# snakers4/silero-vad

Hardware: AMD Instinct MI355X
Metric: audio-chunks/sec (32 ms @ 16 kHz) (higher is better)
Workload: dtype f32; 1 GPU; configs[1]: synthetic 16 kHz PCM resident in HBM, 512-sample chunks, 4096 streams/GPU x 256 chunks/stream per step, zero initial state; streams_per_gpu=4096

## Files before the change

### silero_vad_amd/csrc/fft_wave.hpp

```cpp
#pragma once
#include <hip/hip_runtime.h>

#include "device_api.hpp"
#include "layout.hpp"

#ifndef VAD_NT_PCM
#define VAD_NT_PCM 0
#endif

namespace vad {
namespace {

using f32x4 = float __attribute__((ext_vector_type(4)));
using u32x4 = unsigned __attribute__((ext_vector_type(4)));

#ifndef VAD_TRACE
#define VAD_TRACE 0
#endif
#ifndef VAD_ABLATE
#define VAD_ABLATE 0
#endif

__device__ constexpr float kCos32[16] = {1.0f, 0.98078525f, 0.9238795f, 0.8314696f, 0.70710677f,
    0.55557024f, 0.38268343f, 0.19509032f, 0.0f, -0.19509032f, -0.38268343f, -0.55557024f,
    -0.70710677f, -0.8314696f, -0.9238795f, -0.98078525f};
__device__ constexpr float kSin32[16] = {0.0f, 0.19509032f, 0.38268343f, 0.55557024f, 0.70710677f,
    0.8314696f, 0.9238795f, 0.98078525f, 1.0f, 0.98078525f, 0.9238795f, 0.8314696f, 0.70710677f,
    0.55557024f, 0.38268343f, 0.19509032f};

constexpr int bitrev(int x, int bits) {
    int r = 0;
    for (int i = 0; i < bits; ++i) r |= ((x >> i) & 1) << (bits - 1 - i);
    return r;
}
constexpr int ilog2(int x) { return x <= 1 ? 0 : 1 + ilog2(x / 2); }

struct Lane {
    int lane, g, j, wave;
    long t;
    long tl;
    long st;
    int b;
    bool tile_valid;
    bool from_tail;
    float sgnA, sgnB;
#if VAD_TRACE
    mutable unsigned long long ts[20] = {};
#endif
};
#if VAD_TRACE
#define VAD_WAVE_STAMP(ln, slot) do { (ln).ts[(slot)] = __builtin_readcyclecounter(); } while (0)
#else
#define VAD_WAVE_STAMP(ln, slot) do { } while (0)
#endif

__device__ __forceinline__ void cvt8(const u32x4 v, float *o) {
#pragma unroll
    for (int k = 0; k < 4; ++k) {
        const int lo = (int)(v[k] << 16) >> 16, hi = (int)v[k] >> 16;
        o[2 * k] = (float)lo * (1.0f / 32768.0f);
        o[2 * k + 1] = (float)hi * (1.0f / 32768.0f);
    }
}
template <int SL, int DEC>
__device__ __forceinline__ void load_vec(const float *p, float (&s)[SL]) {
    if (DEC == 1) {
#pragma unroll
        for (int k = 0; k < SL / 4; ++k) {
            const f32x4 v = VAD_NT_PCM ? __builtin_nontemporal_load(reinterpret_cast<const f32x4 *>(p) + k)
                                       : reinterpret_cast<const f32x4 *>(p)[k];
#pragma unroll
            for (int e = 0; e < 4; ++e) s[4 * k + e] = v[e];
        }
    } else {
#pragma unroll
        for (int i = 0; i < SL; ++i) s[i] = p[i * DEC];
        __builtin_amdgcn_sched_barrier(0);
    }
}
template <int SL, int DEC>
__device__ __forceinline__ void load_vec(const int16_t *p, float (&s)[SL]) {
    if (DEC == 1) {
#pragma unroll
        for (int k = 0; k < SL / 8; ++k)
            cvt8(VAD_NT_PCM ? __builtin_nontemporal_load(reinterpret_cast<const u32x4 *>(p) + k)
                            : reinterpret_cast<const u32x4 *>(p)[k], &s[8 * k]);
    } else {
#pragma unroll
        for (int h = 0; h < 2; ++h) {
#pragma unroll
            for (int i = h * SL / 2; i < (h + 1) * SL / 2; ++i) s[i] = (float)p[i * DEC] * (1.0f / 32768.0f);
            __builtin_amdgcn_sched_barrier(0);
        }
    }
}

template <int Q, typename PcmT, int DEC>
__device__ __forceinline__ void load_slice(float (&s)[2 * Q], const FrontArgs &a, const Lane &ln, const int V) {
    constexpr int SL = 2 * Q, N = 16 * Q;
    const PcmT *row = reinterpret_cast<const PcmT *>(a.pcm) + (size_t)ln.b * a.ld;
    const int sigma = 2 * V + ln.g;
    const int sg = (V == 3 && sigma > 8) ? 8 : sigma;
    const long p0 = (long)SL * (8 * ln.t - 1 + sg);
    const PcmT *src = row + p0 * DEC;
    const PcmT *esrc = row + ((long)N * ln.t + N - SL - 1) * DEC;
    if (ln.from_tail) {
        const PcmT *trow = reinterpret_cast<const PcmT *>(a.tail) + (size_t)ln.b * N * DEC;
        if (sg > 0) src = trow + SL * (sg - 1) * DEC;
        esrc = trow + (N - SL - 1) * DEC;
    }
    if (VAD_ABLATE & 16) {
        const PcmT *r0 = reinterpret_cast<const PcmT *>(a.pcm) + (size_t)(ln.st * 16) * a.ld + (long)SL * 8 * ln.t;
#pragma unroll
        for (int k = 0; k < SL / 4; ++k) {
            const f32x4 v = *reinterpret_cast<const f32x4 *>(reinterpret_cast<const float *>(r0) + (size_t)(k & 15) * a.ld + ln.lane * 4);
#pragma unroll
            for (int e = 0; e < 4; ++e) s[4 * k + e] = v[e];
        }
    } else if (VAD_ABLATE & 32) {
        const float *rr = reinterpret_cast<const float *>(row) + (long)SL * 8 * ln.t;
#pragma unroll
        for (int k = 0; k < SL / 4; ++k) {
            const f32x4 v = *reinterpret_cast<const f32x4 *>(rr + 16 * k + 4 * ln.g + 128 * V);
#pragma unroll
            for (int e = 0; e < 4; ++e) s[4 * k + e] = v[e];
        }
    } else if (DEC == 1) {
        if (V == 0 && ln.t == 0 && ln.g == 0) load_vec<SL, 1>(a.ctx_in + (size_t)ln.b * SL, s);
        else load_vec<SL, 1>(src, s);
    } else if (V == 0) {
        const bool from_ctx = ln.t == 0 && ln.g == 0;
        const PcmT *safe = ln.from_tail ? reinterpret_cast<const PcmT *>(a.tail) + (size_t)ln.b * N * DEC : row;
        load_vec<SL, DEC>(from_ctx ? safe : src, s);
        const f32x4 *c4 = reinterpret_cast<const f32x4 *>(a.ctx_in + (size_t)ln.b * SL);
#pragma unroll
        for (int k = 0; k < SL / 4; ++k) {
            const f32x4 v = c4[k];
#pragma unroll
            for (int e = 0; e < 4; ++e) s[4 * k + e] = from_ctx ? v[e] : s[4 * k + e];
        }
    } else {
        load_vec<SL, DEC>(src, s);
    }
    if (V == 3) {
        if (a.ctx_out && ln.t == a.T - 1 && ln.g == 2 && ln.tile_valid &&
            (ln.st * 16 + ln.j) < a.B) {
            float *o = a.ctx_out + (size_t)ln.b * SL;
#pragma unroll
            for (int k = 0; k < SL / 4; ++k)
                reinterpret_cast<f32x4 *>(o)[k] = f32x4{s[4 * k], s[4 * k + 1], s[4 * k + 2], s[4 * k + 3]};
        }
        const bool rev = ln.g == 3;
        float extra = 0.f;
        if (rev) extra = load_pcm(esrc);
#pragma unroll
        for (int i = 0; i < SL / 2 - 1; ++i) {
            const int k = SL - 2 - i;
            const float lo = s[i], hi = s[k];
            s[i] = rev ? hi : lo;
            s[k] = rev ? lo : hi;
        }
        s[SL - 1] = rev ? extra : s[SL - 1];
    }
}

using f32x2 = float __attribute__((ext_vector_type(2)));

__device__ __forceinline__ f32x2 swap2(f32x2 v) { return f32x2{v.y, v.x}; }
__device__ __forceinline__ f32x2 cmul(f32x2 v, float c, float sn) {
    return __builtin_elementwise_fma(swap2(v), f32x2{-sn, sn}, v * f32x2{c, c});
}

#ifndef VAD_XLANE_SWAP
#define VAD_XLANE_SWAP 1
#endif
__device__ __forceinline__ void trade32(f32x2 &a, f32x2 &b) {
#pragma unroll
    for (int e = 0; e < 2; ++e) {
        const auto r = __builtin_amdgcn_permlane32_swap(__float_as_uint(a[e]), __float_as_uint(b[e]), false, false);
        a[e] = __uint_as_float(r[0]);
        b[e] = __uint_as_float(r[1]);
    }
}
__device__ __forceinline__ void trade16(f32x2 &a, f32x2 &b) {
#pragma unroll
    for (int e = 0; e < 2; ++e) {
        const auto r = __builtin_amdgcn_permlane16_swap(__float_as_uint(a[e]), __float_as_uint(b[e]), false, false);
        a[e] = __uint_as_float(r[0]);
        b[e] = __uint_as_float(r[1]);
    }
}

template <int Q>
__device__ __forceinline__ void fft_inlane(f32x2 (&z)[Q]) {
#pragma unroll
    for (int n = Q; n >= 2; n >>= 1) {
        const int half = n >> 1;
#pragma unroll
        for (int b0 = 0; b0 < Q; b0 += n) {
#pragma unroll
            for (int jx = 0; jx < half; ++jx) {
                const int i0 = b0 + jx, i1 = i0 + half;
                const f32x2 u = z[i0], v = z[i1];
                z[i0] = u + v;
                const f32x2 d = u - v;
                const int tw = jx * (32 / n);
                if (tw == 0) z[i1] = d;
                else if (tw == 8) z[i1] = swap2(d) * f32x2{1.0f, -1.0f};
                else z[i1] = cmul(d, kCos32[tw], -kSin32[tw]);
            }
        }
    }
}

template <int Q>
__device__ __forceinline__ void fft_math(float (&X)[Q + 1], const float (&s)[2 * Q], const float *tab_lds, const Lane &ln);

template <int Q, typename PcmT, int DEC = 1>
__device__ __forceinline__ void fft_frame(float (&X)[Q + 1], const int V, const FrontArgs &a, const float *tab_lds,
                                          const Lane &ln) {
    constexpr int SL = 2 * Q;
    __builtin_amdgcn_sched_barrier(0);
    VAD_WAVE_STAMP(ln, 16 + V);
    float s[SL];
    if (VAD_ABLATE & 4) {
#pragma unroll
        for (int i = 0; i < SL; ++i) s[i] = (float)(ln.lane + i) * 1e-3f;
    } else {
        load_slice<Q, PcmT, DEC>(s, a, ln, V);
    }
#if VAD_TRACE
    asm volatile("s_waitcnt vmcnt(0)" ::: "memory");
    VAD_WAVE_STAMP(ln, 2 + 2 * V);
#endif
    if (VAD_ABLATE & 2) {
#pragma unroll
        for (int k = 0; k < Q; ++k) X[k] = s[k] + s[k + Q];
        X[Q] = s[0];
        return;
    }
    fft_math<Q>(X, s, tab_lds, ln);
    VAD_WAVE_STAMP(ln, 3 + 2 * V);
}

template <int Q>
__device__ __forceinline__ void fft_math(float (&X)[Q + 1], const float (&s)[2 * Q], const float *tab_lds, const Lane &ln) {
    constexpr int SL = 2 * Q;
    constexpr vadl::Tab tb = vadl::make_tab(8 * Q, Q);

    f32x2 z[Q];
    {
        const f32x4 *w = reinterpret_cast<const f32x4 *>(tab_lds + tb.window + SL * ln.g);
#pragma unroll
        for (int k = 0; k < SL / 4; ++k) {
            const f32x4 wv = w[k];
            z[2 * k] = f32x2{s[4 * k], s[4 * k + 1]} * f32x2{wv[0], wv[1]};
            z[2 * k + 1] = f32x2{s[4 * k + 2], s[4 * k + 3]} * f32x2{wv[2], wv[3]};
        }
    }
    const f32x4 *tw1 = reinterpret_cast<const f32x4 *>(tab_lds + tb.tw1 + ln.g * Q * 4);
#if VAD_XLANE_SWAP
    constexpr int H = Q / 2;
    const f32x2 rotA = (ln.g & 1) ? f32x2{0.f, 0.f} : f32x2{1.f, 1.f};
    const f32x2 rotB = (ln.g & 1) ? f32x2{1.f, -1.f} : f32x2{0.f, 0.f};
#pragma unroll
    for (int q = 0; q < H; ++q) trade32(z[q], z[q + H]);
#pragma unroll
    for (int q = 0; q < H; ++q) {
        const f32x2 u = z[q], v = z[q + H], d = u - v;
        z[q] = u + v;
        z[q + H] = __builtin_elementwise_fma(swap2(d), rotB, d * rotA);
    }
#pragma unroll
    for (int q = 0; q < H; ++q) trade32(z[q], z[q + H]);
#pragma unroll
    for (int q = 0; q < H; ++q) trade16(z[q], z[q + H]);
#pragma unroll
    for (int q = 0; q < H; ++q) {
        const f32x2 u = z[q], v = z[q + H];
        z[q] = u + v;
        z[q + H] = u - v;
    }
#pragma unroll
    for (int q = 0; q < H; ++q) trade16(z[q], z[q + H]);
#pragma unroll
    for (int q = 0; q < Q; ++q) {
        const f32x2 x = z[q];
        const f32x4 t = tw1[q];
        z[q] = __builtin_elementwise_fma(swap2(x), f32x2{t[0], t[1]}, x * f32x2{t[2], t[2]});
    }
#else
    const f32x2 sA{ln.sgnA, ln.sgnA}, sB{ln.sgnB, ln.sgnB};
    const f32x2 rotA = ln.g == 3 ? f32x2{0.f, 0.f} : f32x2{1.f, 1.f};
    const f32x2 rotB = ln.g == 3 ? f32x2{1.f, -1.f} : f32x2{0.f, 0.f};
#pragma unroll
    for (int q = 0; q < Q; ++q) {
        f32x2 x = z[q];
        const f32x2 p{__shfl_xor(x.x, 32), __shfl_xor(x.y, 32)};
        x = __builtin_elementwise_fma(sA, x, p);
        x = __builtin_elementwise_fma(swap2(x), rotB, x * rotA);
        const f32x2 r{__shfl_xor(x.x, 16), __shfl_xor(x.y, 16)};
        x = __builtin_elementwise_fma(sB, x, r);
        const f32x4 t = tw1[q];
        z[q] = __builtin_elementwise_fma(swap2(x), f32x2{t[0], t[1]}, x * f32x2{t[2], t[2]});
    }
#endif
    fft_inlane<Q>(z);
    constexpr int LG = ilog2(Q);
    const f32x4 *tw2 = reinterpret_cast<const f32x4 *>(tab_lds + tb.tw2 + ln.g * Q * 4);
    const int src_lane4 = (ln.g >= 2 ? (ln.lane ^ 16) : ln.lane) * 4;
#pragma unroll
    for (int k = 0; k < Q; ++k) {
        const f32x2 u = z[bitrev(k, LG)];
        const int ks = bitrev((Q - k) % Q, LG), kr = bitrev(Q - 1 - k, LG);
        const f32x2 own = z[kr], alt = z[ks];
        const float xr = __int_as_float(__builtin_amdgcn_ds_bpermute(src_lane4, __float_as_int(own.x)));
        const float xi = __int_as_float(__builtin_amdgcn_ds_bpermute(src_lane4, __float_as_int(own.y)));
        const f32x2 p{ln.g == 0 ? alt.x : xr, ln.g == 0 ? alt.y : xi};
        const f32x2 av = __builtin_elementwise_fma(p, f32x2{1.0f, -1.0f}, u);
        const f32x2 ev = __builtin_elementwise_fma(p, f32x2{-1.0f, 1.0f}, u);
        const f32x4 t = tw2[k];
        const f32x2 y = __builtin_elementwise_fma(swap2(ev), f32x2{t[0], t[1]},
                                                  __builtin_elementwise_fma(ev, f32x2{t[2], t[2]}, av));
        const f32x2 yy = y * y;
        X[k] = 0.5f * __builtin_amdgcn_sqrtf(yy.x + yy.y);
    }
    X[Q] = ln.g == 0 ? fabsf(z[0].x - z[0].y) : 0.f;
}

template <int Q>
__device__ __forceinline__ void poison_acc(float &p0, float &p1, const float (&X)[Q + 1]) {
#pragma unroll
    for (int k = 0; k < Q; k += 2) {
        p0 = fmaf(X[k], 0.f, p0);
        p1 = fmaf(X[k + 1], 0.f, p1);
    }
}
__device__ __forceinline__ float poison_nyq(float p0, float p1, float xn0, float xn1, float xn2, float xn3) {
    p0 = fmaf(xn0, 0.f, p0);
    p1 = fmaf(xn1, 0.f, p1);
    p0 = fmaf(xn2, 0.f, p0);
    p1 = fmaf(xn3, 0.f, p1);
    return p0 + p1;
}
__device__ __forceinline__ void poison_into(f32x4 &v, float p) {
    v[0] = __uint_as_float(__float_as_uint(v[0]) | __float_as_uint(p));
}

template <int Q, int V, typename PcmT, int DEC = 1>
__device__ __forceinline__ void fft_pass(float (&X)[Q + 1], const FrontArgs &a, const float *tab_lds, const Lane &ln) {
    fft_frame<Q, PcmT, DEC>(X, V, a, tab_lds, ln);
}

}
}
```

### silero_vad_amd/csrc/kernel_front_f43.hip

```cpp
#include <hip/hip_runtime.h>

#include <type_traits>

#include "fft_wave.hpp"
#include "exact_front.hpp"
#include "front_common.hpp"

namespace vad {
namespace {

#ifndef VAD_BV_BATCH
#define VAD_BV_BATCH 1
#endif
constexpr int kUnitBytes = (int)vadl::kWUnitFloats * 4;
struct Ring {
    unsigned a_cur, a_nxt, a_far;
    unsigned d_cur, d_nxt, d_far;
    const float *src;
    unsigned voff;
    f32x4 c0, c1;
};

__device__ __forceinline__ void ring_request(Ring &r) {
    if (VAD_ABLATE & 8) return;
    unsigned keep_m0;
    asm volatile("s_mov_b32 %0, m0\n\ts_mov_b32 m0, %3\n\ts_nop 0\n\t"
                 "global_load_lds_dwordx4 %1, %2\n\tglobal_load_lds_dwordx4 %1, %2 offset:1024\n\t"
                 "global_load_lds_dwordx4 %1, %2 offset:2048\n\tglobal_load_lds_dwordx4 %1, %2 offset:3072\n\t"
                 "s_mov_b32 m0, %0"
                 : "=&s"(keep_m0) : "v"(r.voff), "s"(r.src), "s"(r.d_far) : "memory");
    r.src += vadl::kWUnitFloats;
}
__device__ __forceinline__ void ring_rotate(Ring &r) {
    const unsigned a = r.a_cur, d = r.d_cur;
    r.a_cur = r.a_nxt; r.a_nxt = r.a_far; r.a_far = a;
    r.d_cur = r.d_nxt; r.d_nxt = r.d_far; r.d_far = d;
}

template <int M, int KG, int AFTER, class BF>
__device__ __forceinline__ void gemm_r(f32x4 (&acc)[M], BF bfun, Ring &r) {
    constexpr int NSTEPS = KG * (M / 2), NU = NSTEPS / 8;
    static_assert(NSTEPS % 8 == 0 && M % 2 == 0, "segments are whole units");
    static_for<0, NU>([&](auto uc) VAD_INLINE {
        constexpr int u = decltype(uc)::value, after = (NU - 1 - u) + AFTER;
        static_for<0, 8>([&](auto sc_) VAD_INLINE {
            constexpr int st = decltype(sc_)::value;
            if constexpr (st == 4 && after >= 1) {
                asm volatile("s_waitcnt vmcnt(0)" ::: "memory");
                if (!(VAD_ABLATE & 1)) __builtin_amdgcn_s_barrier();
                asm volatile("" ::: "memory");
                if constexpr (after >= 2) ring_request(r);
            }
            f32x4 n0 = r.c0, n1 = r.c1;
            if constexpr (st + 1 < 8) {
                n0 = lds4(r.a_cur + (2 * (st + 1)) * 1024);
                n1 = lds4(r.a_cur + (2 * (st + 1) + 1) * 1024);
            } else if constexpr (after >= 1) {
                n0 = lds4(r.a_nxt);
                n1 = lds4(r.a_nxt + 1024);
            }
            __builtin_amdgcn_sched_barrier(0);
            constexpr int i = u * 8 + st, kg = i / (M / 2), mp = 2 * (i % (M / 2));
#if VAD_BV_BATCH
            float bv[4];
#pragma unroll
            for (int ks = 0; ks < 4; ++ks) bv[ks] = bfun(kg * 4 + ks);
            __builtin_amdgcn_sched_barrier(0);
#pragma unroll
            for (int ks = 0; ks < 4; ++ks) {
                acc[mp + 0] = __builtin_amdgcn_mfma_f32_16x16x4f32(r.c0[ks], bv[ks], acc[mp + 0], 0, 0, 0);
                acc[mp + 1] = __builtin_amdgcn_mfma_f32_16x16x4f32(r.c1[ks], bv[ks], acc[mp + 1], 0, 0, 0);
            }
#else
#pragma unroll
            for (int ks = 0; ks < 4; ++ks) {
                const float bv = bfun(kg * 4 + ks);
                acc[mp + 0] = __builtin_amdgcn_mfma_f32_16x16x4f32(r.c0[ks], bv, acc[mp + 0], 0, 0, 0);
                acc[mp + 1] = __builtin_amdgcn_mfma_f32_16x16x4f32(r.c1[ks], bv, acc[mp + 1], 0, 0, 0);
            }
#endif
            __builtin_amdgcn_sched_barrier(0);
            r.c0 = n0;
            r.c1 = n1;
        });
        ring_rotate(r);
    });
}

#ifndef VAD_F43_GEMM_PRIO
#define VAD_F43_GEMM_PRIO 0
#endif
#ifndef VAD_F43_FFT_PRIO
#define VAD_F43_FFT_PRIO 0
#endif
template <int Q, typename PcmT, int DEC>
__global__ void __launch_bounds__(256, 2) front_f43_kernel(const FrontArgs a) {
    using namespace vadl;
    constexpr Tab tb = make_tab(8 * Q, Q);
    constexpr int TABF = (tb.total + 3) / 4 * 4;
    constexpr int RB = w_rb(Q), P = w_parts(Q), KG0 = Q / 4;
    constexpr int PB = Q == 32 ? 2 : 1;
    static_assert(w4_tail0(Q) + 20 == w4_units(Q) && P % PB == 0, "program mismatch");
    __shared__ __attribute__((aligned(16))) float lds[TABF + 3 * (kUnitBytes / 4)];
    float *tab = lds;

    Lane ln;
    ln.lane = threadIdx.x & 63;
    ln.wave = __builtin_amdgcn_readfirstlane(threadIdx.x >> 6);
    ln.g = ln.lane >> 4;
    ln.j = ln.lane & 15;
    const long nst = (a.B + 15) / 16, total = nst * a.nt;
    long wt = (long)blockIdx.x * 4 + ln.wave;
    ln.tile_valid = wt < total;
    if (!ln.tile_valid) wt = total - 1;
    ln.tl = wt % a.nt;
    ln.st = wt / a.nt;
    ln.t = a.t0 + ln.tl;
    const long bb = ln.st * 16 + ln.j;
    ln.b = (int)(bb < a.B ? bb : a.B - 1);
    ln.from_tail = a.tail != nullptr && ln.t == a.T - 1;
    ln.sgnA = ln.g < 2 ? 1.f : -1.f;
    ln.sgnB = (ln.g & 1) ? -1.f : 1.f;
#if VAD_TRACE
    VAD_WAVE_STAMP(ln, 0);
#endif

    Ring ring;
    {
        const unsigned slot0 = (unsigned)(size_t)((__attribute__((address_space(3))) float *)(lds + TABF));
        ring.voff = ln.lane * 16;
        ring.a_cur = slot0 + ring.voff;
        ring.a_nxt = ring.a_cur + kUnitBytes;
        ring.a_far = ring.a_cur + 2 * kUnitBytes;
        ring.d_far = slot0 + (unsigned)ln.wave * 4096u;
        ring.d_cur = ring.d_far + kUnitBytes;
        ring.d_nxt = ring.d_far + 2 * kUnitBytes;
        ring.src = a.wfront + ln.wave * 1024;
        ring_request(ring);
        {   const unsigned d = ring.d_far; ring.d_far = ring.d_cur; ring.d_cur = ring.d_nxt; ring.d_nxt = d; }
        ring_request(ring);
        {   const unsigned d = ring.d_far; ring.d_far = ring.d_cur; ring.d_cur = ring.d_nxt; ring.d_nxt = d; }
    }
    {
        static_assert(tb.total % 4 == 0, "tables are copied as 16-byte vectors");
        constexpr int NV = tb.total / 4, PER = (NV + 255) / 256;
        const f32x4 *src = reinterpret_cast<const f32x4 *>(a.tables);
        f32x4 v[PER];
#pragma unroll
        for (int k = 0; k < PER; ++k) {
            const int i = threadIdx.x + k * 256;
            v[k] = src[i < NV ? i : NV - 1];
        }
#pragma unroll
        for (int k = 0; k < PER; ++k) {
            const int i = threadIdx.x + k * 256;
            if (i < NV) reinterpret_cast<f32x4 *>(tab)[i] = v[k];
        }
    }
    asm volatile("s_waitcnt vmcnt(0)" ::: "memory");
    __syncthreads();
    VAD_WAVE_STAMP(ln, 1);

    float X0[Q + 1], X1[Q + 1], X2[Q + 1], X3[Q + 1];
#pragma unroll
    for (int k = 0; k <= Q; ++k) X1[k] = X2[k] = X3[k] = 0.f;
#pragma clang loop unroll(disable)
    for (int v = 0; v < 4; ++v) {
        if (v >= 3) {
#pragma unroll
            for (int k = 0; k <= Q; ++k) X0[k] = X1[k];
        }
        if (v >= 2) {
#pragma unroll
            for (int k = 0; k <= Q; ++k) X1[k] = X2[k];
        }
        if (v >= 1) {
#pragma unroll
            for (int k = 0; k <= Q; ++k) X2[k] = X3[k];
        }
        if (VAD_F43_FFT_PRIO) __builtin_amdgcn_s_setprio(VAD_F43_FFT_PRIO);
        fft_frame<Q, PcmT, DEC>(X3, v, a, tab, ln);
        if (VAD_F43_FFT_PRIO) __builtin_amdgcn_s_setprio(0);
    }
    if (VAD_F43_GEMM_PRIO) __builtin_amdgcn_s_setprio(VAD_F43_GEMM_PRIO);
    const float xn0 = __shfl(X0[Q], ln.j), xn1 = __shfl(X1[Q], ln.j), xn2 = __shfl(X2[Q], ln.j), xn3 = __shfl(X3[Q], ln.j);
    if (!VAD_NO_EXACT && a.exact_list != nullptr) {
        const SilentMasks sm = silent_chunks(X0[0], X1[0], X2[0], X3[0]);
        const long left = (long)a.B - ln.st * 16;
        const unsigned take = (sm.edge | (a.gx_silent != nullptr ? sm.silent : 0u)) & (left >= 16 ? 0xffffu : ((1u << left) - 1u));
        if (take != 0 && ln.tile_valid) {
            int base = 0;
            if (ln.lane == 0) base = atomicAdd(a.exact_list, __builtin_popcount(take));
            base = __shfl(base, 0);
            if (ln.g == 0 && ((take >> ln.j) & 1))
                a.exact_list[2 + base + __builtin_popcount(take & ((1u << ln.j) - 1u))] =
                    (int)(wt * 16 + ln.j) | (((sm.silent >> ln.j) & 1) ? kExactSilentBit : 0);
        }
    }

#if VAD_F43_EF
#pragma unroll
    for (int k = 0; k < Q; ++k) {
        X3[k] = X3[k] - X1[k];
        X0[k] = X2[k] - X0[k];
    }
    float poison;
    {   float p0 = 0.f, p1 = 0.f;
        poison_acc<Q>(p0, p1, X3);
        poison_acc<Q>(p0, p1, X0);
        poison = poison_nyq(p0, p1, xn0, xn1, xn2, xn3);
    }
#else
    float poison;
    {   float p0 = 0.f, p1 = 0.f;
        poison_acc<Q>(p0, p1, X0);
        poison_acc<Q>(p0, p1, X1);
        poison_acc<Q>(p0, p1, X2);
        poison_acc<Q>(p0, p1, X3);
        poison = poison_nyq(p0, p1, xn0, xn1, xn2, xn3);
    }
#endif
    ring.c0 = lds4(ring.a_cur);
    ring.c1 = lds4(ring.a_cur + 1024);

    f32x4 Z0[4], Z1[4];
    zero<4>(Z0);
    zero<4>(Z1);
#pragma clang loop unroll(disable)
    for (int it = 0; it < P / PB; ++it) {
        f32x4 Ykeep[RB];
        static_for<0, PB>([&](auto pc) VAD_INLINE {
            constexpr int pb = decltype(pc)::value;
            const int row0 = 16 * RB * (it * PB + pb);
            const float *wn = tab + tb.w_nyq + row0;
            f32x4 Y0[RB], Y1[RB], Y2[RB], Y3[RB];
            zero<RB>(Y0);
            zero<RB>(Y1);
            zero<RB>(Y2);
            zero<RB>(Y3);
#if VAD_F43_EF
            {   const Coef k = opaque_coef<kF4, kFm3>();
                gemm_r<RB, KG0, 2>(Y0, [&](int s) VAD_INLINE {
                    return fmaf(fmaf(X2[s], k.p1, X1[s]), k.b, fmaf(X0[s], k.a, X3[s])); }, ring);
                const Coef k2 = opaque_coef<kFm4, kF3>();
                gemm_r<RB, KG0, 2>(Y1, [&](int s) VAD_INLINE {
                    return fmaf(fmaf(X1[s], k2.m1, X2[s]), k2.b, fmaf(X0[s], k2.a, X3[s])); }, ring);
            }
            {   const Coef k = opaque_coef<kF2, kFm2>();
                gemm_r<RB, KG0, 2>(Y2, [&](int s) VAD_INLINE { return fmaf(X0[s], k.a, X3[s]); }, ring);
                gemm_r<RB, KG0, 2>(Y3, [&](int s) VAD_INLINE { return fmaf(X0[s], k.b, X3[s]); }, ring);
            }
#else
            {   const Coef k = opaque_coef<kFm4, kF4>();
                gemm_r<RB, KG0, 2>(Y0, [&](int s) VAD_INLINE {
                    return fmaf(fmaf(X1[s], k.p1, X0[s]), k.a, fmaf(X3[s], k.p1, X2[s])); }, ring);
                gemm_r<RB, KG0, 2>(Y1, [&](int s) VAD_INLINE {
                    return fmaf(fmaf(X1[s], k.m1, X0[s]), k.b, fmaf(X2[s], k.m1, X3[s])); }, ring);
            }
            {   const Coef k = opaque_coef<kF2, kFm2>();
                gemm_r<RB, KG0, 2>(Y2, [&](int s) VAD_INLINE {
                    return fmaf(fmaf(X0[s], k.m1, X2[s]), k.a, fmaf(X1[s], k.m1, X3[s])); }, ring);
                const Coef k2 = opaque_coef<kF2, kFm2>();
                gemm_r<RB, KG0, 2>(Y3, [&](int s) VAD_INLINE {
                    return fmaf(fmaf(X0[s], k2.m1, X2[s]), k2.b, fmaf(X1[s], k2.m1, X3[s])); }, ring);
            }
#endif
#pragma unroll
            for (int m = 0; m < RB; ++m)
#pragma unroll
                for (int r = 0; r < 4; ++r) {
                    const float sm = Y0[m][r] + Y1[m][r], df = Y0[m][r] - Y1[m][r];
                    const float s2 = Y2[m][r] + Y3[m][r], d2 = Y2[m][r] - Y3[m][r];
                    Y0[m][r] = sm + s2;
                    Y1[m][r] = fmaf(2.f, d2, df);
                    Y2[m][r] = fmaf(4.f, s2, sm);
                    Y3[m][r] = fmaf(8.f, d2, df);
                }
#if VAD_F43_EF
            {   const Coef k = opaque_coef<kFm4, kFm025>();
                gemm_r<RB, KG0, 2>(Y0, [&](int s) VAD_INLINE { return fmaf(X1[s], k.a, X3[s]); }, ring);
                gemm_r<RB, KG0, 2>(Y3, [&](int s) VAD_INLINE { return fmaf(X2[s], k.b, -X0[s]); }, ring);
            }
#else
            {   const Coef k = opaque_coef<kFm5, kFm125>();
                gemm_r<RB, KG0, 2>(Y0, [&](int s) VAD_INLINE { return fmaf(X1[s], k.a, X3[s]); }, ring);
                gemm_r<RB, KG0, 2>(Y3, [&](int s) VAD_INLINE { return fmaf(X2[s], k.b, X0[s]); }, ring);
            }
#endif
            nyq_update<RB>(Y0, xn0, wn + 128, ln);
            nyq_update<RB>(Y0, xn1, wn + 256, ln);
            nyq_update<RB>(Y1, xn0, wn, ln);
            nyq_update<RB>(Y1, xn1, wn + 128, ln);
            nyq_update<RB>(Y1, xn2, wn + 256, ln);
            nyq_update<RB>(Y2, xn1, wn, ln);
            nyq_update<RB>(Y2, xn2, wn + 128, ln);
            nyq_update<RB>(Y2, xn3, wn + 256, ln);
            nyq_update<RB>(Y3, xn2, wn, ln);
            nyq_update<RB>(Y3, xn3, wn + 128, ln);
            add_bias<RB>(Y0, tab + tb.b_e0 + row0, ln);
            add_bias<RB>(Y1, tab + tb.b_e0 + row0, ln);
            add_bias<RB>(Y2, tab + tb.b_e0 + row0, ln);
            add_bias<RB>(Y3, tab + tb.b_e0 + row0, ln);
            relu<RB>(Y0);
            relu<RB>(Y1);
            relu<RB>(Y2);
            relu<RB>(Y3);
            if constexpr (Q == 32) {
                auto two = [](const f32x4 (&A)[RB], const f32x4 (&B)[RB], int s) VAD_INLINE {
                    return s < 8 ? A[s >> 2][s & 3] : B[(s - 8) >> 2][s & 3];
                };
                gemm_r<4, 4, 2>(Z0, [&](int s) VAD_INLINE { return two(Y0, Y1, s); }, ring);
                gemm_r<4, 4, 2>(Z1, [&](int s) VAD_INLINE { return two(Y1, Y2, s); }, ring);
                if constexpr (pb == 0) {
#pragma unroll
                    for (int m = 0; m < RB; ++m) Ykeep[m] = Y3[m];
                } else {
                    gemm_r<4, 4, 2>(Z1, [&](int s) VAD_INLINE { return two(Ykeep, Y3, s); }, ring);
                }
            } else {
                auto one = [](const f32x4 (&A)[RB], int s) VAD_INLINE { return A[s >> 2][s & 3]; };
                gemm_r<4, 4, 2>(Z0, [&](int s) VAD_INLINE { return one(Y0, s); }, ring);
                gemm_r<4, 4, 2>(Z0, [&](int s) VAD_INLINE { return one(Y1, s); }, ring);
                gemm_r<4, 4, 2>(Z1, [&](int s) VAD_INLINE { return one(Y1, s); }, ring);
                gemm_r<4, 4, 2>(Z1, [&](int s) VAD_INLINE { return one(Y2, s); }, ring);
                gemm_r<4, 4, 2>(Z1, [&](int s) VAD_INLINE { return one(Y3, s); }, ring);
            }
        });
    }
    add_bias<4>(Z0, tab + tb.b_e1, ln);
    add_bias<4>(Z1, tab + tb.b_e1, ln);
    relu<4>(Z0);
    relu<4>(Z1);
    VAD_WAVE_STAMP(ln, 10);

    f32x4 Vv[4];
    auto bZ0 = [&](int s) VAD_INLINE { return Z0[s >> 2][s & 3]; };
    auto bZ1 = [&](int s) VAD_INLINE { return Z1[s >> 2][s & 3]; };
    auto bV = [&](int s) VAD_INLINE { return Vv[s >> 2][s & 3]; };
    init_bias<4>(Vv, tab + tb.b_e2, ln);
    gemm_r<4, 4, 2>(Vv, bZ0, ring);
    gemm_r<4, 4, 2>(Vv, bZ1, ring);
    relu<4>(Vv);
    f32x4 Fe[8];
    auto bF = [&](int s) VAD_INLINE { return Fe[s >> 2][s & 3]; };
    init_bias<8>(Fe, tab + tb.b_e3, ln);
    gemm_r<8, 4, 2>(Fe, bV, ring);
    relu<8>(Fe);
    poison_into(Fe[0], poison);
    VAD_WAVE_STAMP(ln, 11);

    float *gxt = a.gx + ((size_t)(ln.st * a.nt + ln.tl) * 32) * 256 + ln.lane * 4;
    const float *bg = tab + tb.b_g;
#pragma clang loop unroll(disable)
    for (int q = 0; q < 3; ++q) {
        f32x4 G[8];
        init_bias<8>(G, bg, ln);
        gemm_r<8, 8, 2>(G, bF, ring);
        if (ln.tile_valid) {
#pragma unroll
            for (int m = 0; m < 8; ++m) *reinterpret_cast<f32x4 *>(gxt + (size_t)m * 256) = G[m];
        }
        gxt += 8 * 256;
        bg += 128;
    }
    {
        f32x4 G[8];
        init_bias<8>(G, bg, ln);
        gemm_r<8, 8, 0>(G, bF, ring);
        if (ln.tile_valid) {
#pragma unroll
            for (int m = 0; m < 8; ++m) *reinterpret_cast<f32x4 *>(gxt + (size_t)m * 256) = G[m];
        }
    }
#if VAD_TRACE
    VAD_WAVE_STAMP(ln, 12);
    if (a.trace && ln.lane == 0) {
        long long *tr = a.trace + ((size_t)blockIdx.x * 4 + ln.wave) * 32;
#pragma unroll
        for (int k = 0; k < 20; ++k) tr[k] = (long long)ln.ts[k];
        tr[13] = __builtin_amdgcn_s_getreg((31 << 11) | 4);
        tr[14] = __builtin_amdgcn_s_getreg((31 << 11) | 20);
        tr[15] = (long long)wall_clock64();
    }
#endif
}

}

template <typename PcmT>
hipError_t launch_front_f43(int sr, const FrontArgs &a, hipStream_t s) {
    if (a.B <= 0 || a.nt <= 0) return hipSuccess;
    const long nst = (a.B + 15) / 16, total = nst * a.nt;
    const unsigned grid = (unsigned)((total + 3) / 4);
    if (a.dec > 1 && (sr != 16000 || a.dec > 3)) return hipErrorInvalidValue;
    if (a.dec == 3) hipLaunchKernelGGL((front_f43_kernel<32, PcmT, 3>), dim3(grid), dim3(256), 0, s, a);
    else if (a.dec == 2) hipLaunchKernelGGL((front_f43_kernel<32, PcmT, 2>), dim3(grid), dim3(256), 0, s, a);
    else if (sr == 16000) hipLaunchKernelGGL((front_f43_kernel<32, PcmT, 1>), dim3(grid), dim3(256), 0, s, a);
    else hipLaunchKernelGGL((front_f43_kernel<16, PcmT, 1>), dim3(grid), dim3(256), 0, s, a);
    return hipGetLastError();
}
template hipError_t launch_front_f43<float>(int, const FrontArgs &, hipStream_t);
template hipError_t launch_front_f43<int16_t>(int, const FrontArgs &, hipStream_t);

}
```

Before: 189.4 million chunks/s.

## Software-pipeline LDS twiddle/window loads and bpermutes in the FFT front, raise FFT priority

The window, tw1 and tw2 LDS reads and the ds_bpermute exchanges in the per-frame FFT are restructured into batched prefetches with explicit partial lgkmcnt waits, so later batches' LDS traffic overlaps arithmetic on earlier batches. Twiddle rows are loaded as 3-float vectors instead of 4. The FFT wave's priority is now raised only once its PCM global loads have arrived (vmcnt wait inside fft_math), and the default FFT priority becomes 1. This adds register pressure from the staged buffers and depends on hand-coded waitcnt encodings being correct.

```diff
diff --git a/silero_vad_amd/csrc/fft_wave.hpp b/silero_vad_amd/csrc/fft_wave.hpp
--- a/silero_vad_amd/csrc/fft_wave.hpp
+++ b/silero_vad_amd/csrc/fft_wave.hpp
@@ -213,10 +213,10 @@
     }
 }
 
-template <int Q>
+template <int Q, int ARRIVE = -1>
 __device__ __forceinline__ void fft_math(float (&X)[Q + 1], const float (&s)[2 * Q], const float *tab_lds, const Lane &ln);
 
-template <int Q, typename PcmT, int DEC = 1>
+template <int Q, typename PcmT, int DEC = 1, int PRIO = 0>
 __device__ __forceinline__ void fft_frame(float (&X)[Q + 1], const int V, const FrontArgs &a, const float *tab_lds,
                                           const Lane &ln) {
     constexpr int SL = 2 * Q;
@@ -239,26 +239,77 @@
         X[Q] = s[0];
         return;
     }
-    fft_math<Q>(X, s, tab_lds, ln);
+    fft_math<Q, PRIO>(X, s, tab_lds, ln);
+    if (PRIO > 0) __builtin_amdgcn_s_setprio(0);
     VAD_WAVE_STAMP(ln, 3 + 2 * V);
 }
 
-template <int Q>
+__device__ __forceinline__ void lds_fence() { __builtin_amdgcn_sched_barrier(0); }
+template <int N>
+__device__ __forceinline__ void lds_wait() {
+    static_assert(N >= 0 && N <= 15, "lgkmcnt is a 4-bit field");
+    lds_fence();
+    __builtin_amdgcn_s_waitcnt(0xc07f | (N << 8));
+    lds_fence();
+}
+__device__ __forceinline__ void lds_wait_n(int n) {
+    if (n >= 15) lds_wait<15>();
+    else if (n >= 12) lds_wait<12>();
+    else if (n >= 8) lds_wait<8>();
+    else if (n >= 4) lds_wait<4>();
+    else if (n >= 2) lds_wait<2>();
+    else lds_wait<0>();
+}
+template <int N>
+__device__ __forceinline__ void lds_rows(f32x4 (&o)[N], const f32x4 *p) {
+#pragma unroll
+    for (int i = 0; i < N; ++i) o[i] = p[i];
+}
+using f32x3 = float __attribute__((ext_vector_type(3)));
+__device__ __forceinline__ f32x3 tw_row(const f32x4 *p) { return *reinterpret_cast<const f32x3 *>(p); }
+
+template <int Q, int ARRIVE>
 __device__ __forceinline__ void fft_math(float (&X)[Q + 1], const float (&s)[2 * Q], const float *tab_lds, const Lane &ln) {
     constexpr int SL = 2 * Q;
     constexpr vadl::Tab tb = vadl::make_tab(8 * Q, Q);
+    constexpr int TB = 4, NTB = Q / TB, T1B = 4, NT1 = Q / T1B, T1D = 3;
+    static_assert(Q % TB == 0 && SL % 16 == 0, "batches are whole");
+    const f32x4 *tw1 = reinterpret_cast<const f32x4 *>(tab_lds + tb.tw1 + ln.g * Q * 4);
+    const f32x4 *tw2 = reinterpret_cast<const f32x4 *>(tab_lds + tb.tw2 + ln.g * Q * 4);
 
     f32x2 z[Q];
     {
+        constexpr int NWB = 4, WQ = SL / 4 / NWB;
         const f32x4 *w = reinterpret_cast<const f32x4 *>(tab_lds + tb.window + SL * ln.g);
-#pragma unroll
-        for (int k = 0; k < SL / 4; ++k) {
-            const f32x4 wv = w[k];
-            z[2 * k] = f32x2{s[4 * k], s[4 * k + 1]} * f32x2{wv[0], wv[1]};
-            z[2 * k + 1] = f32x2{s[4 * k + 2], s[4 * k + 3]} * f32x2{wv[2], wv[3]};
-        }
-    }
-    const f32x4 *tw1 = reinterpret_cast<const f32x4 *>(tab_lds + tb.tw1 + ln.g * Q * 4);
+        f32x4 wv[NWB][WQ];
+        lds_fence();
+        lds_rows<WQ>(wv[0], w);
+        lds_rows<WQ>(wv[1], w + WQ);
+        if (ARRIVE >= 0) {
+            lds_fence();
+            __builtin_amdgcn_s_waitcnt(0x0f70);
+            if (ARRIVE > 0) __builtin_amdgcn_s_setprio(ARRIVE);
+        }
+#pragma unroll
+        for (int b = 0; b < NWB; ++b) {
+            if (b < NWB - 1) lds_wait<WQ>();
+            else lds_wait<0>();
+#pragma unroll
+            for (int i = 0; i < WQ; ++i) {
+                const int k = b * WQ + i;
+                z[2 * k] = f32x2{s[4 * k], s[4 * k + 1]} * f32x2{wv[b][i][0], wv[b][i][1]};
+                z[2 * k + 1] = f32x2{s[4 * k + 2], s[4 * k + 3]} * f32x2{wv[b][i][2], wv[b][i][3]};
+            }
+            lds_fence();
+            if (b + 2 < NWB) lds_rows<WQ>(wv[b + 2], w + (b + 2) * WQ);
+        }
+    }
+    f32x3 t1[NT1][T1B];
+#pragma unroll
+    for (int b = 0; b < T1D - 1; ++b)
+#pragma unroll
+        for (int i = 0; i < T1B; ++i) t1[b][i] = tw_row(tw1 + b * T1B + i);
+    lds_fence();
 #if VAD_XLANE_SWAP
     constexpr int H = Q / 2;
     const f32x2 rotA = (ln.g & 1) ? f32x2{0.f, 0.f} : f32x2{1.f, 1.f};
@@ -283,12 +334,6 @@
     }
 #pragma unroll
     for (int q = 0; q < H; ++q) trade16(z[q], z[q + H]);
-#pragma unroll
-    for (int q = 0; q < Q; ++q) {
-        const f32x2 x = z[q];
-        const f32x4 t = tw1[q];
-        z[q] = __builtin_elementwise_fma(swap2(x), f32x2{t[0], t[1]}, x * f32x2{t[2], t[2]});
-    }
 #else
     const f32x2 sA{ln.sgnA, ln.sgnA}, sB{ln.sgnB, ln.sgnB};
     const f32x2 rotA = ln.g == 3 ? f32x2{0.f, 0.f} : f32x2{1.f, 1.f};
@@ -300,32 +345,76 @@
         x = __builtin_elementwise_fma(sA, x, p);
         x = __builtin_elementwise_fma(swap2(x), rotB, x * rotA);
         const f32x2 r{__shfl_xor(x.x, 16), __shfl_xor(x.y, 16)};
-        x = __builtin_elementwise_fma(sB, x, r);
-        const f32x4 t = tw1[q];
-        z[q] = __builtin_elementwise_fma(swap2(x), f32x2{t[0], t[1]}, x * f32x2{t[2], t[2]});
-    }
-#endif
+        z[q] = __builtin_elementwise_fma(sB, x, r);
+    }
+#endif
+    lds_fence();
+#pragma unroll
+    for (int b = 0; b < NT1; ++b) {
+        if (b + T1D - 1 < NT1) {
+#pragma unroll
+            for (int i = 0; i < T1B; ++i) t1[b + T1D - 1][i] = tw_row(tw1 + (b + T1D - 1) * T1B + i);
+        }
+        lds_wait_n((NT1 - 1 - b < T1D - 1 ? NT1 - 1 - b : T1D - 1) * T1B);
+#pragma unroll
+        for (int i = 0; i < T1B; ++i) {
+            const int q = b * T1B + i;
+            const f32x2 x = z[q];
+            const f32x3 t = t1[b][i];
+            z[q] = __builtin_elementwise_fma(swap2(x), f32x2{t[0], t[1]}, x * f32x2{t[2], t[2]});
+        }
+        lds_fence();
+    }
+    constexpr int LG = ilog2(Q);
+    const int src_lane4 = (ln.g >= 2 ? (ln.lane ^ 16) : ln.lane) * 4;
+    f32x3 t2[NTB][TB];
+    float xr[NTB][TB], xi[NTB][TB];
+    auto bin = [&](int n, int i) { return i < TB / 2 ? (TB / 2) * n + i : Q - 1 - (TB / 2) * n - (i - TB / 2); };
+    auto rows = [&](int n) __attribute__((always_inline)) {
+#pragma unroll
+        for (int i = 0; i < TB; ++i) t2[n][i] = tw_row(tw2 + bin(n, i));
+    };
+    auto fetch = [&](int n) __attribute__((always_inline)) {
+#pragma unroll
+        for (int i = 0; i < TB; ++i) {
+            const f32x2 own = z[bitrev(Q - 1 - bin(n, i), LG)];
+            xr[n][i] = __int_as_float(__builtin_amdgcn_ds_bpermute(src_lane4, __float_as_int(own.x)));
+            xi[n][i] = __int_as_float(__builtin_amdgcn_ds_bpermute(src_lane4, __float_as_int(own.y)));
+        }
+    };
+    rows(0);
+    lds_fence();
     fft_inlane<Q>(z);
-    constexpr int LG = ilog2(Q);
-    const f32x4 *tw2 = reinterpret_cast<const f32x4 *>(tab_lds + tb.tw2 + ln.g * Q * 4);
-    const int src_lane4 = (ln.g >= 2 ? (ln.lane ^ 16) : ln.lane) * 4;
-#pragma unroll
-    for (int k = 0; k < Q; ++k) {
-        const f32x2 u = z[bitrev(k, LG)];
-        const int ks = bitrev((Q - k) % Q, LG), kr = bitrev(Q - 1 - k, LG);
-        const f32x2 own = z[kr], alt = z[ks];
-        const float xr = __int_as_float(__builtin_amdgcn_ds_bpermute(src_lane4, __float_as_int(own.x)));
-        const float xi = __int_as_float(__builtin_amdgcn_ds_bpermute(src_lane4, __float_as_int(own.y)));
-        const f32x2 p{ln.g == 0 ? alt.x : xr, ln.g == 0 ? alt.y : xi};
-        const f32x2 av = __builtin_elementwise_fma(p, f32x2{1.0f, -1.0f}, u);
-        const f32x2 ev = __builtin_elementwise_fma(p, f32x2{-1.0f, 1.0f}, u);
-        const f32x4 t = tw2[k];
-        const f32x2 y = __builtin_elementwise_fma(swap2(ev), f32x2{t[0], t[1]},
-                                                  __builtin_elementwise_fma(ev, f32x2{t[2], t[2]}, av));
-        const f32x2 yy = y * y;
-        X[k] = 0.5f * __builtin_amdgcn_sqrtf(yy.x + yy.y);
-    }
     X[Q] = ln.g == 0 ? fabsf(z[0].x - z[0].y) : 0.f;
+    lds_fence();
+    fetch(0);
+#pragma unroll
+    for (int n = 0; n < NTB; ++n) {
+        if (n + 1 < NTB) {
+            rows(n + 1);
+            fetch(n + 1);
+            lds_wait<3 * TB>();
+        } else {
+            lds_wait<0>();
+        }
+        float m2[TB];
+#pragma unroll
+        for (int i = 0; i < TB; ++i) {
+            const int k = bin(n, i);
+            const f32x2 u = z[bitrev(k, LG)], alt = z[bitrev((Q - k) % Q, LG)];
+            const f32x2 p{ln.g == 0 ? alt.x : xr[n][i], ln.g == 0 ? alt.y : xi[n][i]};
+            const f32x2 av = __builtin_elementwise_fma(p, f32x2{1.0f, -1.0f}, u);
+            const f32x2 ev = __builtin_elementwise_fma(p, f32x2{-1.0f, 1.0f}, u);
+            const f32x3 t = t2[n][i];
+            const f32x2 y = __builtin_elementwise_fma(swap2(ev), f32x2{t[0], t[1]},
+                                                      __builtin_elementwise_fma(ev, f32x2{t[2], t[2]}, av));
+            const f32x2 yy = y * y;
+            m2[i] = yy.x + yy.y;
+        }
+#pragma unroll
+        for (int i = 0; i < TB; ++i) X[bin(n, i)] = 0.5f * __builtin_amdgcn_sqrtf(m2[i]);
+        lds_fence();
+    }
 }
 
 template <int Q>
diff --git a/silero_vad_amd/csrc/kernel_front_f43.hip b/silero_vad_amd/csrc/kernel_front_f43.hip
--- a/silero_vad_amd/csrc/kernel_front_f43.hip
+++ b/silero_vad_amd/csrc/kernel_front_f43.hip
@@ -91,7 +91,7 @@
 #define VAD_F43_GEMM_PRIO 0
 #endif
 #ifndef VAD_F43_FFT_PRIO
-#define VAD_F43_FFT_PRIO 0
+#define VAD_F43_FFT_PRIO 1
 #endif
 template <int Q, typename PcmT, int DEC>
 __global__ void __launch_bounds__(256, 2) front_f43_kernel(const FrontArgs a) {
@@ -178,9 +178,7 @@
 #pragma unroll
             for (int k = 0; k <= Q; ++k) X2[k] = X3[k];
         }
-        if (VAD_F43_FFT_PRIO) __builtin_amdgcn_s_setprio(VAD_F43_FFT_PRIO);
-        fft_frame<Q, PcmT, DEC>(X3, v, a, tab, ln);
-        if (VAD_F43_FFT_PRIO) __builtin_amdgcn_s_setprio(0);
+        fft_frame<Q, PcmT, DEC, VAD_F43_FFT_PRIO>(X3, v, a, tab, ln);
     }
     if (VAD_F43_GEMM_PRIO) __builtin_amdgcn_s_setprio(VAD_F43_GEMM_PRIO);
     const float xn0 = __shfl(X0[Q], ln.j), xn1 = __shfl(X1[Q], ln.j), xn2 = __shfl(X2[Q], ln.j), xn3 = __shfl(X3[Q], ln.j);
```

Result: faster. 194.4 million chunks/s, median of 6 (+2.6%).
